# unknownue/puflow

Hardware: AMD Instinct MI355X
Metric: patches/sec x4 2048->8192 (PU1K discrete, eval) (higher is better)
Workload: dtype f32 (split-fp16 MFMA products, fp32 accumulate); 1 GPU; BASELINE configs[1]: PU1K discrete x4 inference, 32 x 2048-pt patches per GPU (fp32-parity mode); patches_per_gpu=32, total_batch=32, npoint=2048

## Files before the change

puflow_amd/csrc/edgeconv.hip:

```cpp
#include <hip/hip_runtime.h>
#include "pf_api_internal.h"
#include "pf_mfma.h"

#if defined(__HIP_DEVICE_COMPILE__)
#define PF_PACKED_FP32_FN __attribute__((target("packed-fp32-ops")))
#else
#define PF_PACKED_FP32_FN
#endif

namespace {

struct EcArgs {
    const float* pq;
    const float* xyz;
    const float* tab;
    const int* idx;
    const f4* wg;
    float* out;
    int T;
    int N;
    int chunk;
    int ntiles;
    const u4* pqf_w;
    const float* pqf_bias;
    const float* pqf_scales;
    float* pqf_out;
};

template <int ODIM>
__device__ __forceinline__ void pqf_stage(u4* hb, int ch, int pt, float v) {
    _Float16* h = reinterpret_cast<_Float16*>(hb);
    const int cp = ch >> 5, j = ((ch >> 4) & 1) * 4 + (ch & 3), slot = 16 * ((ch & 15) >> 2) + pt;
    const _Float16 hi = (_Float16)v;
    const _Float16 lo = (_Float16)(v - (float)hi);
    h[((cp * 2 + 0) * 64 + slot) * 8 + j] = hi;
    h[((cp * 2 + 1) * 64 + slot) * 8 + j] = lo;
}

constexpr int PQF_NT = 4;

template <int ODIM, int ROWS, int NW>
__device__ __forceinline__ void pqf_gemm(const EcArgs& a, const u4* hb, int nst, const int (&tpt)[PQF_NT], int wave_u, int lane) {
    constexpr int CP = ODIM / 32, RB = ROWS / 16 / NW;
    static_assert(ODIM % 32 == 0 && ROWS % (16 * NW) == 0, "rows split evenly over the waves");
    constexpr int OBW = NW <= 8 ? RB : 1;
    const int col = lane & 15, q = lane >> 4;
    const PfW2BufD<CP> ws(a.pqf_w, lane);
    const float inv = a.pqf_scales[6];
#pragma unroll
    for (int ob0 = 0; ob0 < RB; ob0 += OBW) {
        h8 wh[OBW][CP], wl[OBW][CP];
#pragma unroll
        for (int o = 0; o < OBW; ++o)
#pragma unroll
            for (int cp = 0; cp < CP; ++cp) {
                wh[o][cp] = ws.load((wave_u * RB + ob0 + o) * CP + cp, 0);
                wl[o][cp] = ws.load((wave_u * RB + ob0 + o) * CP + cp, 1);
            }
#pragma unroll
        for (int t = 0; t < PQF_NT; ++t) {
            if (t >= nst) break;
            const u4* hbt = hb + t * (CP * 2 * 64);
            f4 acc[OBW];
#pragma unroll
            for (int o = 0; o < OBW; ++o) acc[o] = pf_splat(0.f);
#pragma unroll
            for (int cp = 0; cp < CP; ++cp) {
                const h8 fh = __builtin_bit_cast(h8, hbt[(cp * 2 + 0) * 64 + lane]), fl = __builtin_bit_cast(h8, hbt[(cp * 2 + 1) * 64 + lane]);
#pragma unroll
                for (int o = 0; o < OBW; ++o) {
                    f4 x = acc[o];
                    if constexpr (PF_MMN_TERMS == 3) {
                        x = pf_mfma_f16(wh[o][cp], fl, x);
                        x = pf_mfma_f16(wl[o][cp], fh, x);
                    }
                    x = pf_mfma_f16(wh[o][cp], fh, x);
                    acc[o] = x;
                }
            }
            const int pt = tpt[t] + col;
            if (pt < a.T) {
#pragma unroll
                for (int o = 0; o < OBW; ++o) {
                    const f4 bias = *reinterpret_cast<const f4*>(a.pqf_bias + (wave_u * RB + ob0 + o) * 16 + 4 * q);
                    f4 v;
#pragma unroll
                    for (int r = 0; r < 4; ++r) v[r] = fmaf(acc[o][r], inv, bias[r]);
                    *reinterpret_cast<f4*>(a.pqf_out + (size_t)pt * ROWS + (wave_u * RB + ob0 + o) * 16 + 4 * q) = v;
                }
            }
        }
    }
}

struct PqfState {
    int nst = 0;
    int tpt[PQF_NT] = {0, 0, 0, 0};
    __device__ __forceinline__ void push(int pt0) {
#pragma unroll
        for (int k = 0; k < PQF_NT; ++k) tpt[k] = k == nst ? pt0 : tpt[k];
        ++nst;
    }
};

template <int GB, int NCONV, int ODIM, bool C3, int P, int NW>
__global__ __launch_bounds__(NW * 64) void edgeconv_kernel(EcArgs a) {
    constexpr int G = GB * 16;
    constexpr int S = G * NCONV + ODIM;
    constexpr int NF = GB * NCONV;
    constexpr int OBO = ODIM / 16;
    constexpr int OCH = 2;
    static_assert(OBO <= 16 && OBO % OCH == 0, "pooled store uses one lane column per output block");
    const int lane = threadIdx.x & 63, wave = threadIdx.x >> 6;
    const int col = lane & 15, q = lane >> 4;

    constexpr int NWF = GB * GB * (NCONV * (NCONV - 1) / 2) + OBO * NF;
    __shared__ f4 wlds[NWF * 64];
    pf_stage_lds(wlds, a.wg, NWF * 64);
    __syncthreads();
    const PfWLds ws{wlds, lane};

    for (int v = blockIdx.x; v < 8 * a.chunk; v += gridDim.x) {
        const int tile = pf_xcd_tile(v, a.chunk);
        if (tile >= a.ntiles) continue;
        const int pt0 = (tile * NW + wave) * P;

        int gi[P], gj[P];
        float xi[P][3], xj[P][3];
#pragma unroll
        for (int p = 0; p < P; ++p) {
            int g = pt0 + p;
            g = g < a.T ? g : a.T - 1;
            gi[p] = g;
            const int b = g / a.N;
            gj[p] = b * a.N + a.idx[(size_t)g * 16 + col];
            if constexpr (C3) {
#pragma unroll
                for (int c = 0; c < 3; ++c) {
                    xi[p][c] = a.xyz[(size_t)gi[p] * 3 + c];
                    xj[p][c] = a.xyz[(size_t)gj[p] * 3 + c];
                }
            }
        }

        auto init = [&](int p, int off) -> f4 {
            if constexpr (C3) {
                f4 r;
#pragma unroll
                for (int k = 0; k < 4; ++k) {
                    const f4* t = reinterpret_cast<const f4*>(a.tab + (size_t)(off + k) * 8);
                    const f4 t0 = t[0], t1 = t[1];
                    float s = t1.z;
                    s = fmaf(t0.x, xi[p][0], s); s = fmaf(t0.y, xi[p][1], s); s = fmaf(t0.z, xi[p][2], s);
                    s = fmaf(t0.w, xj[p][0], s); s = fmaf(t1.x, xj[p][1], s); s = fmaf(t1.y, xj[p][2], s);
                    r[k] = s;
                }
                return r;
            } else {
                const f4 pv = *reinterpret_cast<const f4*>(a.pq + (size_t)gi[p] * (2 * S) + off);
                const f4 qv = *reinterpret_cast<const f4*>(a.pq + (size_t)gj[p] * (2 * S) + S + off);
                return pv + qv;
            }
        };

        constexpr int NI = GB > OCH ? GB : OCH;
        f4 ini[2][P][NI];
        auto load_init = [&](auto nbc, int row0, f4 (&dst)[P][NI]) {
            constexpr int NB = decltype(nbc)::value;
#pragma unroll
            for (int ob = 0; ob < NB; ++ob)
#pragma unroll
                for (int p = 0; p < P; ++p) dst[p][ob] = init(p, row0 + ob * 16 + 4 * q);
        };
        using IGB = std::integral_constant<int, GB>;
        using IOC = std::integral_constant<int, OCH>;
        load_init(IGB{}, 0, ini[0]);
        if constexpr (NCONV > 1) load_init(IGB{}, G, ini[1]); else load_init(IOC{}, G * NCONV, ini[1]);

        f4 feat[P][NF];
#pragma unroll
        for (int ob = 0; ob < GB; ++ob)
#pragma unroll
            for (int p = 0; p < P; ++p) feat[p][ob] = pf_lrelu(ini[0][p][ob], 0.05f);

        pf_static_for<1, NCONV>([&](auto tc) {
            constexpr int t = decltype(tc)::value;
            if constexpr (t + 1 < NCONV) load_init(IGB{}, G * (t + 1), ini[(t + 1) & 1]);
            else load_init(IOC{}, G * NCONV, ini[(t + 1) & 1]);
            f4 acc[P][GB];
#pragma unroll
            for (int ob = 0; ob < GB; ++ob)
#pragma unroll
                for (int p = 0; p < P; ++p) acc[p][ob] = ini[t & 1][p][ob];
            pf_mm<GB, GB * t, GB * t>(ws, GB * GB * (t * (t - 1) / 2), feat, 0, acc, 0);
#pragma unroll
            for (int ob = 0; ob < GB; ++ob)
#pragma unroll
                for (int p = 0; p < P; ++p) feat[p][GB * t + ob] = pf_lrelu(acc[p][ob], 0.05f);
        });

        constexpr int FO = GB * GB * (NCONV * (NCONV - 1) / 2);
        f4 sel[P];
#pragma unroll
        for (int p = 0; p < P; ++p) sel[p] = pf_splat(0.f);
        pf_static_for<0, OBO / OCH>([&](auto cc) {
            constexpr int c = decltype(cc)::value;
            constexpr int ob0 = c * OCH;
            constexpr int st = NCONV + c;
            if constexpr (c + 1 < OBO / OCH) load_init(IOC{}, G * NCONV + (ob0 + OCH) * 16, ini[(st + 1) & 1]);
            f4 acc[P][OCH];
#pragma unroll
            for (int o = 0; o < OCH; ++o)
#pragma unroll
                for (int p = 0; p < P; ++p) acc[p][o] = ini[st & 1][p][o];
            pf_mm<OCH, NF, NF>(ws, FO + ob0 * NF, feat, 0, acc, 0);
#pragma unroll
            for (int o = 0; o < OCH; ++o)
#pragma unroll
                for (int p = 0; p < P; ++p) {
                    f4 m;
#pragma unroll
                    for (int r = 0; r < 4; ++r) m[r] = pf_rowmax16(acc[p][o][r]);
                    if (col == ob0 + o) sel[p] = m;
                }
        });
#pragma unroll
        for (int p = 0; p < P; ++p)
            if (col < OBO && pt0 + p < a.T)
                *reinterpret_cast<f4*>(a.out + (size_t)gi[p] * ODIM + col * 16 + 4 * q) = sel[p];
    }
}

struct EcWConst {
    static constexpr int DEPTH = 2;
    int lane;
    __device__ __forceinline__ h8 load(int frag, int split) const {
        const _Float16 x = (_Float16)(float)((lane + frag + split) & 7);
        return (h8){x, x, x, x, x, x, x, x};
    }
};

constexpr float EC4_OUT_INV = 1.f / 256.f;

template <int P, int NW, int DBG = 0, bool PQF = false>
__global__ __launch_bounds__(NW * 64) PF_PACKED_FP32_FN void edgeconv4_kernel(EcArgs a) {
    static_assert(!PQF || NW * P == 16, "the fused P|Q GEMM takes a workgroup tile of 16 points as one MFMA column tile");
    constexpr int NCONV = 4, G = 32, S = 256, OBO = 8, OCH = 2, ODIM = 128;
    constexpr int NWF = 2 * (NCONV * (NCONV - 1) / 2) + OBO * NCONV;
    constexpr int ROWB = 2 * S * 4;
    const int lane = threadIdx.x & 63, wave = threadIdx.x >> 6;
    const int col = lane & 15, q = lane >> 4;
    __shared__ u4 wlds[NWF * 2 * 64];
    __shared__ f4 plds[NW * P][64];
    __shared__ u4 hb[PQF ? PQF_NT * (ODIM / 32) * 2 * 64 : 1];
    PqfState pqf;
    pf_stage_lds(wlds, reinterpret_cast<const u4*>(a.wg), NWF * 2 * 64);
    __syncthreads();
    const PfW2Lds ws_lds{wlds, lane};
    const auto ws = [&] { if constexpr ((DBG & 4) != 0) return EcWConst{lane}; else return ws_lds; }();
    const __amdgpu_buffer_rsrc_t rs = __builtin_amdgcn_make_buffer_rsrc(const_cast<float*>(a.pq), 0, 0x7fffffff, 0x00020000);
    const int blkq = ((q & 1) << 1) | (q >> 1);

    const int vend = 8 * a.chunk;
    auto next_valid = [&](int v) { while (v < vend && pf_xcd_tile(v, a.chunk) >= a.ntiles) v += gridDim.x; return v; };
    struct Pre { int g[P]; int jc[P]; int4 j4[P]; f4 prow[P]; };
    auto fetch = [&](int v, Pre& n) {
        const int pt0 = (pf_xcd_tile(v < vend ? v : blockIdx.x, a.chunk) * NW + wave) * P;
#pragma unroll
        for (int p = 0; p < P; ++p) {
            int g = pt0 + p;
            g = g < a.T ? g : a.T - 1;
            g = __builtin_amdgcn_readfirstlane(g);
            n.g[p] = g;
            n.jc[p] = a.idx[(size_t)g * 16 + col];
            n.j4[p] = *reinterpret_cast<const int4*>(a.idx + (size_t)g * 16 + 4 * q);
            n.prow[p] = __builtin_bit_cast(f4, __builtin_amdgcn_raw_buffer_load_b128(rs, lane * 16, g * ROWB, 0));
        }
    };
    int v = next_valid(blockIdx.x);
    Pre cur;
    if (v < vend) fetch(v, cur);
    while (v < vend) {
        const int pt0 = (pf_xcd_tile(v, a.chunk) * NW + wave) * P;
        const int vn = next_valid(v + gridDim.x);
        int vQ[P];
        int vO[P][4];
        int gout[P];
#pragma unroll
        for (int p = 0; p < P; ++p) {
            const int g = cur.g[p];
            const int bN = (g / a.N) * a.N;
            gout[p] = g;
            plds[wave * P + p][lane] = cur.prow[p];
            vQ[p] = (bN + cur.jc[p]) * ROWB + (S + 4 * q) * 4;
            vO[p][0] = (bN + cur.j4[p].x) * ROWB + (S + G * NCONV + col) * 4;
            vO[p][1] = (bN + cur.j4[p].y) * ROWB + (S + G * NCONV + col) * 4;
            vO[p][2] = (bN + cur.j4[p].z) * ROWB + (S + G * NCONV + col) * 4;
            vO[p][3] = (bN + cur.j4[p].w) * ROWB + (S + G * NCONV + col) * 4;
        }
        fetch(vn, cur);
        auto load_g = [&](int t, f4 (&dst)[P][2]) {
#pragma unroll
            for (int ob = 0; ob < 2; ++ob)
#pragma unroll
                for (int p = 0; p < P; ++p) {
                    const int off = (G * t + 16 * ob) * 4;
                    if constexpr (DBG & 1) { dst[p][ob] = pf_splat((float)(off + vQ[p]) * 1e-9f); continue; }
                    dst[p][ob] = __builtin_bit_cast(f4, __builtin_amdgcn_raw_buffer_load_b128(rs, vQ[p], off, 0));
                }
        };
        auto p_g = [&](int p, int t, int ob) -> f4 { return plds[wave * P + p][(G * t + 16 * ob) / 4 + q]; };
        auto load_o = [&](int ob0, f4 (&dst)[P][2]) {
#pragma unroll
            for (int o = 0; o < OCH; ++o)
#pragma unroll
                for (int p = 0; p < P; ++p)
#pragma unroll
                    for (int r = 0; r < 4; ++r) {
                        if constexpr (DBG & 1) { dst[p][o][r] = (float)(vO[p][r] + ob0 + o) * 1e-9f; continue; }
                        dst[p][o][r] = __builtin_bit_cast(float, __builtin_amdgcn_raw_buffer_load_b32(rs, vO[p][r], (ob0 + o) * 64, 0));
                    }
        };
        f4 ini[2][P][2];
        load_g(0, ini[0]);
        load_g(1, ini[1]);
        PfPairN feat[P][NCONV];
#pragma unroll
        for (int p = 0; p < P; ++p)
            feat[p][0] = pf_pairn(pf_lrelu(ini[0][p][0] + p_g(p, 0, 0), 0.05f), pf_lrelu(ini[0][p][1] + p_g(p, 0, 1), 0.05f));
        pf_static_for<1, NCONV>([&](auto tc) {
            constexpr int t = decltype(tc)::value;
            if constexpr (t + 1 < NCONV) load_g(t + 1, ini[(t + 1) & 1]); else load_o(0, ini[(t + 1) & 1]);
            f4 acc[P][2];
#pragma unroll
            for (int ob = 0; ob < 2; ++ob)
#pragma unroll
                for (int p = 0; p < P; ++p) acc[p][ob] = ini[t & 1][p][ob] + p_g(p, t, ob);
            if constexpr (!(DBG & 2)) pf_mmn<false, 2, t, t>(ws, 2 * (t * (t - 1) / 2), feat, acc);
#pragma unroll
            for (int p = 0; p < P; ++p) {
                if constexpr (DBG & 8) { feat[p][t] = feat[p][0]; feat[p][t].h[0] += (_Float16)acc[p][0].x; continue; }
                feat[p][t] = pf_pairn(pf_lrelu(acc[p][0], 0.05f), pf_lrelu(acc[p][1], 0.05f));
            }
        });
        constexpr int FO = 2 * (NCONV * (NCONV - 1) / 2);
        float m[P][OBO];
        pf_static_for<0, OBO / OCH>([&](auto cc) {
            constexpr int c = decltype(cc)::value;
            constexpr int ob0 = c * OCH;
            constexpr int st = NCONV + c;
            if constexpr (c + 1 < OBO / OCH) load_o(ob0 + OCH, ini[(st + 1) & 1]);
            f4 acc[P][OCH];
#pragma unroll
            for (int o = 0; o < OCH; ++o)
#pragma unroll
                for (int p = 0; p < P; ++p) acc[p][o] = ini[st & 1][p][o];
            if constexpr (!(DBG & 2)) pf_mmn<true, OCH, NCONV, NCONV>(ws, FO + ob0 * NCONV, feat, acc);
#pragma unroll
            for (int o = 0; o < OCH; ++o)
#pragma unroll
                for (int p = 0; p < P; ++p)
                    m[p][ob0 + o] = fmaxf(fmaxf(acc[p][o].x, acc[p][o].y), fmaxf(acc[p][o].z, acc[p][o].w));
        });
#pragma unroll
        for (int p = 0; p < P; ++p) {
            const float o0 = pf_rsmax16(pf_rsmax32(m[p][0], m[p][1]), pf_rsmax32(m[p][2], m[p][3]));
            const float o1 = pf_rsmax16(pf_rsmax32(m[p][4], m[p][5]), pf_rsmax32(m[p][6], m[p][7]));
            const int ch = 16 * blkq + col;
            const float* pr = reinterpret_cast<const float*>(plds[wave * P + p]);
            const float p0 = pr[G * NCONV + ch], p1 = pr[G * NCONV + 64 + ch];
            const float h0 = fmaf(o0, EC4_OUT_INV, p0), h1 = fmaf(o1, EC4_OUT_INV, p1);
            if (pt0 + p < a.T) {
                float* o = a.out + (size_t)gout[p] * ODIM + ch;
                o[0] = h0;
                o[64] = h1;
            }
            if constexpr (PQF) {
                u4* hbt = hb + pqf.nst * ((ODIM / 32) * 2 * 64);
                pqf_stage<ODIM>(hbt, ch, wave * P + p, h0);
                pqf_stage<ODIM>(hbt, ch + 64, wave * P + p, h1);
            }
        }
        if constexpr (PQF) {
            pqf.push(pf_xcd_tile(v, a.chunk) * NW * P);
            if (pqf.nst == PQF_NT || vn >= vend) {
                __syncthreads();
                pqf_gemm<ODIM, 2 * S, NW>(a, hb, pqf.nst, pqf.tpt, __builtin_amdgcn_readfirstlane(wave), lane);
                __syncthreads();
                pqf.nst = 0;
            }
        }
        v = vn;
    }
}

template <int P, int NW, int DBG = 0, bool PQF = false>
int launch4(const EcArgs& a0, hipStream_t s) {
    EcArgs a = a0;
    a.ntiles = (a.T + NW * P - 1) / (NW * P);
    a.chunk = (a.ntiles + 7) / 8;
    int grid = 8 * a.chunk;
    if (grid > 256) grid = 256;
    hipLaunchKernelGGL((edgeconv4_kernel<P, NW, DBG, PQF>), dim3(grid), dim3(NW * 64), 0, s, a);
    return pf_last_launch_status();
}

template <int ODIM, bool C3, int P, int NW, bool PQF = false>
__global__ __launch_bounds__(NW * 64) void edgeconv1n_kernel(EcArgs a) {
    static_assert(!PQF || NW * P == 16, "the fused P|Q GEMM takes a workgroup tile of 16 points as one MFMA column tile");
    constexpr int NCONV = 4, S = 16 * NCONV + ODIM, SB = S / 16, OBO = ODIM / 16;
    constexpr int PQ_ROWS = ODIM == 32 ? 256 : 512;
    constexpr int FO = 4, FT = FO + OBO * 2, NWF = FT + (C3 ? SB / 2 : 0);
    static_assert(!C3 || SB % 2 == 0, "the edge table fills whole 2-KiB slots");
    constexpr int ROWB = 2 * S * 4;
    static_assert(OBO == 2 || OBO == 4, "reduce-scatter below is written for 2 or 4 output blocks");
    const int lane = threadIdx.x & 63, wave = threadIdx.x >> 6;
    const int col = lane & 15, q = lane >> 4;
    __shared__ u4 wlds[NWF * 128];
    __shared__ float plds[C3 ? 1 : NW * P][C3 ? 1 : S];
    __shared__ u4 hb[PQF ? PQF_NT * (ODIM / 32) * 2 * 64 : 1];
    PqfState pqf;
    pf_stage_lds(wlds, reinterpret_cast<const u4*>(a.wg), NWF * 128);
    __syncthreads();
    const PfW2Lds ws{wlds, lane};
    const float inv_tab = C3 ? reinterpret_cast<const float*>(a.wg)[NWF * 512] : 1.f;
    const __amdgpu_buffer_rsrc_t rs = __builtin_amdgcn_make_buffer_rsrc(const_cast<float*>(C3 ? a.xyz : a.pq), 0, 0x7fffffff, 0x00020000);

    for (int v = blockIdx.x; v < 8 * a.chunk; v += gridDim.x) {
        const int tile = pf_xcd_tile(v, a.chunk);
        if (tile >= a.ntiles) continue;
        const int pt0 = (tile * NW + wave) * P;
        int gi[P], vQ[P], vO[P][4];
        h8 e[P];
#pragma unroll
        for (int p = 0; p < P; ++p) {
            int g = pt0 + p;
            g = g < a.T ? g : a.T - 1;
            g = __builtin_amdgcn_readfirstlane(g);
            gi[p] = g;
            const int bN = (g / a.N) * a.N;
            const int jc = bN + a.idx[(size_t)g * 16 + col];
            if constexpr (C3) {
                float xi[3], xj[3];
#pragma unroll
                for (int c = 0; c < 3; ++c) {
                    xi[c] = a.xyz[(size_t)g * 3 + c];
                    xj[c] = a.xyz[(size_t)jc * 3 + c];
                }
                const f4 e0 = {xi[0], xi[1], xi[2], xj[0]}, e1 = {xj[1], xj[2], 0.f, 1.f};
                e[p] = pf_edge_operand(e0, e1, q);
            } else {
                const int4 j4 = *reinterpret_cast<const int4*>(a.idx + (size_t)g * 16 + 4 * q);
                vQ[p] = jc * ROWB + (S + 4 * q) * 4;
                vO[p][0] = (bN + j4.x) * ROWB + (S + 16 * NCONV + col) * 4;
                vO[p][1] = (bN + j4.y) * ROWB + (S + 16 * NCONV + col) * 4;
                vO[p][2] = (bN + j4.z) * ROWB + (S + 16 * NCONV + col) * 4;
                vO[p][3] = (bN + j4.w) * ROWB + (S + 16 * NCONV + col) * 4;
                if (lane * 2 < S) {
                    typedef float f2 __attribute__((ext_vector_type(2)));
                    const f2 pv = *reinterpret_cast<const f2*>(a.pq + (size_t)g * (2 * S) + lane * 2);
                    *reinterpret_cast<f2*>(&plds[wave * P + p][lane * 2]) = pv;
                }
            }
        }
        f4 pre[P][NCONV];
        f4 outi[P][OBO];
        if constexpr (C3) {
#pragma unroll
            for (int p = 0; p < P; ++p) {
#pragma unroll
                for (int b = 0; b < NCONV; ++b) pre[p][b] = pf_splat(0.f);
#pragma unroll
                for (int b = 0; b < OBO; ++b) outi[p][b] = pf_splat(0.f);
            }
            const PfW1Lds wt{wlds + FT * 128, lane};
            pf_mm1<false, NCONV>(wt, 0, e, pre);
            pf_mm1<true, OBO>(wt, NCONV, e, outi);
#pragma unroll
            for (int p = 0; p < P; ++p) {
#pragma unroll
                for (int b = 0; b < NCONV; ++b) pre[p][b] = pre[p][b] * inv_tab;
#pragma unroll
                for (int b = 0; b < OBO; ++b) outi[p][b] = outi[p][b] * inv_tab;
            }
        } else {
#pragma unroll
            for (int b = 0; b < NCONV; ++b)
#pragma unroll
                for (int p = 0; p < P; ++p)
                    pre[p][b] = __builtin_bit_cast(f4, __builtin_amdgcn_raw_buffer_load_b128(rs, vQ[p], b * 64, 0));
#pragma unroll
            for (int b = 0; b < OBO; ++b)
#pragma unroll
                for (int p = 0; p < P; ++p)
#pragma unroll
                    for (int r = 0; r < 4; ++r)
                        outi[p][b][r] = __builtin_bit_cast(float, __builtin_amdgcn_raw_buffer_load_b32(rs, vO[p][r], b * 64, 0));
#pragma unroll
            for (int b = 0; b < NCONV; ++b)
#pragma unroll
                for (int p = 0; p < P; ++p) pre[p][b] += *reinterpret_cast<const f4*>(&plds[wave * P + p][16 * b + 4 * q]);
        }

        PfPairN fp[P][2];
        PfHalfN last[P];
#pragma unroll
        for (int p = 0; p < P; ++p) {
            last[p] = pf_act_halfn(pre[p][0], 0.05f);
            fp[p][0] = pf_join_halfn(last[p], PfHalfN{});
        }
        pf_static_for<1, NCONV>([&](auto tc) {
            constexpr int t = decltype(tc)::value;
            constexpr int CPT = (t + 1) / 2, F0 = (t / 2) * ((t + 1) / 2);
            f4 acc[P][1];
#pragma unroll
            for (int p = 0; p < P; ++p) acc[p][0] = pre[p][t];
            pf_mmn<false, 1, CPT, CPT>(ws, F0, fp, acc);
#pragma unroll
            for (int p = 0; p < P; ++p) {
                const PfHalfN f = pf_act_halfn(acc[p][0], 0.05f);
                if constexpr (t % 2 == 1) fp[p][t / 2] = pf_join_halfn(last[p], f);
                else fp[p][t / 2] = pf_join_halfn(f, PfHalfN{});
                last[p] = f;
            }
        });
        pf_mmn<true, OBO, 2, 2>(ws, FO, fp, outi);
#pragma unroll
        for (int p = 0; p < P; ++p) {
            float m[OBO];
#pragma unroll
            for (int b = 0; b < OBO; ++b) m[b] = fmaxf(fmaxf(outi[p][b].x, outi[p][b].y), fmaxf(outi[p][b].z, outi[p][b].w));
            float o;
            int ch;
            if constexpr (OBO == 4) {
                o = pf_rsmax16(pf_rsmax32(m[0], m[1]), pf_rsmax32(m[2], m[3]));
                ch = 16 * (((q & 1) << 1) | (q >> 1)) + col;
            } else {
                const float n = pf_rsmax32(m[0], m[1]);
                o = pf_rsmax16(n, n);
                ch = 16 * (q >> 1) + col;
            }
            float pv = 0.f;
            if constexpr (!C3) pv = plds[wave * P + p][16 * NCONV + ch];
            const float hv = fmaf(o, EC4_OUT_INV, pv);
            if (pt0 + p < a.T && (OBO == 4 || (q & 1) == 0))
                a.out[(size_t)gi[p] * ODIM + ch] = hv;
            if constexpr (PQF) {
                if (OBO == 4 || (q & 1) == 0) pqf_stage<ODIM>(hb + pqf.nst * ((ODIM / 32) * 2 * 64), ch, wave * P + p, hv);
            }
        }
        if constexpr (PQF) {
            pqf.push(tile * NW * P);
            if (pqf.nst == PQF_NT) {
                __syncthreads();
                pqf_gemm<ODIM, PQ_ROWS, NW>(a, hb, pqf.nst, pqf.tpt, __builtin_amdgcn_readfirstlane(wave), lane);
                __syncthreads();
                pqf.nst = 0;
            }
        }
    }
    if constexpr (PQF) {
        if (pqf.nst > 0) {
            __syncthreads();
            pqf_gemm<ODIM, PQ_ROWS, NW>(a, hb, pqf.nst, pqf.tpt, __builtin_amdgcn_readfirstlane(wave), lane);
        }
    }
}

template <int ODIM, bool C3, int P, int NW, bool PQF = false>
int launch1n(const EcArgs& a0, hipStream_t s) {
    EcArgs a = a0;
    a.ntiles = (a.T + NW * P - 1) / (NW * P);
    a.chunk = (a.ntiles + 7) / 8;
    int grid = 8 * a.chunk;
    const int cap = 256 * (32 / NW);
    if (grid > cap) grid = cap;
    hipLaunchKernelGGL((edgeconv1n_kernel<ODIM, C3, P, NW, PQF>), dim3(grid), dim3(NW * 64), 0, s, a);
    return pf_last_launch_status();
}

template <int ODIM, bool C3>
int launch1n_v(const EcArgs& a, hipStream_t s, int variant) {
    switch (variant) {
        case 1: return launch1n<ODIM, C3, 2, 8>(a, s);
#ifdef PF_TUNING_VARIANTS
        case 0: return launch1n<ODIM, C3, 1, 8>(a, s);
        case 2: return launch1n<ODIM, C3, 1, 16>(a, s);
        case 3: return launch1n<ODIM, C3, 2, 4>(a, s);
#endif
        default: return PF_ERR_UNSUPPORTED;
    }
}

template <int GB, int NCONV, int ODIM, bool C3, int P, int NW>
int launch_v(const EcArgs& a0, hipStream_t s) {
    EcArgs a = a0;
    a.ntiles = (a.T + NW * P - 1) / (NW * P);
    a.chunk = (a.ntiles + 7) / 8;
    constexpr int NF = GB * NCONV;
    constexpr int lds = (GB * GB * (NCONV * (NCONV - 1) / 2) + (ODIM / 16) * NF) * 1024;
    int per_cu = (160 * 1024) / lds;
    const int by_waves = 32 / NW;
    if (per_cu > by_waves) per_cu = by_waves;
    if (per_cu < 1) per_cu = 1;
    int grid = 8 * a.chunk;
    const int cap = 256 * per_cu;
    if (grid > cap) grid = cap;
    hipLaunchKernelGGL((edgeconv_kernel<GB, NCONV, ODIM, C3, P, NW>), dim3(grid), dim3(NW * 64), 0, s, a);
    return pf_last_launch_status();
}

template <int GB, int NCONV, int ODIM, bool C3>
int launch(const EcArgs& a, hipStream_t s, int variant) {
    constexpr int BEST = ODIM == 32 ? 0 : (ODIM == 64 ? 2 : 3);
    if (variant == BEST) {
        if constexpr (BEST == 0) return launch_v<GB, NCONV, ODIM, C3, 2, 8>(a, s);
        else if constexpr (BEST == 2) return launch_v<GB, NCONV, ODIM, C3, 1, 8>(a, s);
        else return launch_v<GB, NCONV, ODIM, C3, 1, 16>(a, s);
    }
#ifdef PF_TUNING_VARIANTS
    switch (variant) {
        case 0: return launch_v<GB, NCONV, ODIM, C3, 2, 8>(a, s);
        case 1: return launch_v<GB, NCONV, ODIM, C3, 2, 4>(a, s);
        case 2: return launch_v<GB, NCONV, ODIM, C3, 1, 8>(a, s);
        case 3: return launch_v<GB, NCONV, ODIM, C3, 1, 16>(a, s);
        default: break;
    }
#endif
    return PF_ERR_UNSUPPORTED;
}

}

extern "C" int pf_edgeconv_tuned(int cfg, int variant, const float* pq_or_xyz, const float* tab, const int* idx,
                                 const float* wfrag, float* out, int B, int N, void* stream) {
    if (!pq_or_xyz || !idx || !wfrag || !out) return PF_ERR_NULL;
    if (B <= 0 || N < 16 || (long long)B * N > (1ll << 30)) return PF_ERR_SHAPE;
    EcArgs a{};
    a.idx = idx; a.wg = reinterpret_cast<const f4*>(wfrag); a.out = out; a.T = B * N; a.N = N;
    hipStream_t s = (hipStream_t)stream;
    switch (cfg) {
        case 0:
            if (!tab) return PF_ERR_NULL;
            a.xyz = pq_or_xyz; a.tab = tab;
            return launch<1, 4, 32, true>(a, s, variant);
        case 1: a.pq = pq_or_xyz; return launch<1, 4, 64, false>(a, s, variant);
        case 2: a.pq = pq_or_xyz; return launch<2, 4, 128, false>(a, s, variant);
        case 7:
            {
                const long long maxT = 0x7fffffffll / 2048;
                if (N > maxT) return PF_ERR_UNSUPPORTED;
                const int Bc = (int)(maxT / N);
                for (int b0 = 0; b0 < B; b0 += Bc) {
                    const int nb = B - b0 < Bc ? B - b0 : Bc;
                    EcArgs c = a;
                    c.pq = pq_or_xyz + (size_t)b0 * N * 512; c.idx = idx + (size_t)b0 * N * 16; c.out = out + (size_t)b0 * N * 128;
                    c.T = nb * N;
                    int rc;
                    switch (variant) {
                        case 0: rc = launch4<1, 16>(c, s); break;
#ifdef PF_TUNING_VARIANTS
                        case 1: rc = launch4<2, 8>(c, s); break;
                        case 2: rc = launch4<1, 8>(c, s); break;
                        case 3: rc = launch4<2, 4>(c, s); break;
                        case 8: rc = launch4<1, 16, 1>(c, s); break;
                        case 9: rc = launch4<1, 16, 2>(c, s); break;
                        case 10: rc = launch4<1, 16, 4>(c, s); break;
                        case 11: rc = launch4<1, 16, 5>(c, s); break;
                        case 12: rc = launch4<1, 16, 3>(c, s); break;
                        case 13: rc = launch4<1, 16, 6>(c, s); break;
                        case 14: rc = launch4<1, 16, 13>(c, s); break;
#endif
                        default: return PF_ERR_UNSUPPORTED;
                    }
                    if (rc != PF_OK) return rc;
                }
                return PF_OK;
            }
        case 8:
            a.xyz = pq_or_xyz;
            if ((long long)B * N * 12 > 0x7fffffffll) return PF_ERR_SHAPE;
            return launch1n_v<32, true>(a, s, variant);
        case 9:
            a.pq = pq_or_xyz;
            if ((long long)B * N * 1024 > 0x7fffffffll) return PF_ERR_SHAPE;
            return launch1n_v<64, false>(a, s, variant);
        default: return PF_ERR_UNSUPPORTED;
    }
}

extern "C" int pf_edgeconv(int cfg, const float* pq_or_xyz, const float* tab, const int* idx, const float* wfrag,
                           float* out, int B, int N, void* stream) {
    static const int best[10] = {0, 2, 3, -1, -1, -1, -1, 0, 1, 1};
    if (cfg < 0 || cfg > 9 || best[cfg] < 0) return PF_ERR_UNSUPPORTED;
    return pf_edgeconv_tuned(cfg, best[cfg], pq_or_xyz, tab, idx, wfrag, out, B, N, stream);
}

extern "C" int pf_edgeconv_pq(int unit, const float* pq_or_xyz, const int* idx, const float* wfrag, float* out, const float* w,
                              const long long* off, float* pq_next, int B, int N, int fuse, void* stream) {
    if (!pq_or_xyz || !idx || !wfrag || !out || !w || !off || !pq_next) return PF_ERR_NULL;
    if (unit < 0 || unit > 4) return PF_ERR_UNSUPPORTED;
    if (B <= 0 || N < 16 || (long long)B * N > (1ll << 30)) return PF_ERR_SHAPE;
    const long long T = (long long)B * N;
    const bool fits32 = unit == 0 ? T * 12 <= 0x7fffffffll : (unit == 1 ? T * 1024 <= 0x7fffffffll : T * 2048 <= 0x7fffffffll);
    const bool fused = fits32 && (fuse == 1 || (fuse < 0 && T <= 16384));
    const int cfg = unit == 0 ? 8 : (unit == 1 ? 9 : 7);
    if (!fused) {
        const int rc = pf_edgeconv(cfg, pq_or_xyz, nullptr, idx, wfrag, out, B, N, stream);
        return rc != PF_OK ? rc : pf_pq_gemm(unit, out, w, off, pq_next, (int)T, stream);
    }
    EcArgs a{};
    a.idx = idx; a.wg = reinterpret_cast<const f4*>(wfrag); a.out = out; a.T = (int)T; a.N = N;
    a.pqf_w = reinterpret_cast<const u4*>(w + off[10]); a.pqf_bias = w + off[11]; a.pqf_scales = w + off[12]; a.pqf_out = pq_next;
    hipStream_t s = (hipStream_t)stream;
    if (unit == 0) { a.xyz = pq_or_xyz; return launch1n<32, true, 2, 8, true>(a, s); }
    a.pq = pq_or_xyz;
    if (unit == 1) return launch1n<64, false, 2, 8, true>(a, s);
    return launch4<1, 16, 0, true>(a, s);
}
```

puflow_amd/interpflow.py:

```python
from __future__ import annotations

import os
from typing import List, Optional, Tuple

import numpy as np
import torch
import torch.nn as nn
from torch import Tensor

from . import _lib
from .packing import COND_CHANNELS, FEAT_CHANNELS, GROWTH, NUM_BLOCKS, fold_state_dict, pack_plan

_EC_CFG = [0, 1, 2, 2, 2, 2]
_CHECK_FINITE = os.environ.get("PF_CHECK_FINITE", "0") == "1"


def _conv_bn(cin: int, cout: int, slope: float) -> nn.Sequential:
    return nn.Sequential(nn.Conv2d(cin, cout, kernel_size=1), nn.BatchNorm2d(cout), nn.LeakyReLU(slope))


class _EdgeConvParams(nn.Module):

    def __init__(self, cin: int, odim: int, growth: int):
        super().__init__()
# ... 104 lines not shown
        self.base = self.blob.data_ptr()
        self.ec_tab0 = pk["ec_tab0"]
        self.ec_w = pk["ec_w"]
        self.ec4_w = pk["ec4_w"]
        self.ec1n_w = pk["ec1n_w"]
        self.post = [_lib.offsets(o) for o in pk["post"]]
        self.post_all = _lib.offsets([v for o in pk["post"] for v in o])
        self.flow = pk["flow"]
        self.interp_off = _lib.offsets(pk["interp"])
        self.ld_const = pk["ld_const"]
        self._logp_ws = {}
        self._side = None
        self.split_interp = 0
        self.fuse_pq = -1

    def _p(self, off: int) -> int:
        return self.base + 4 * off

    def _edgeconv(self, u: int, src: int, idx16: Tensor, h: Tensor, B: int, N: int, s) -> None:
        lib = self.lib
        if self.ec_mode == "f16n":
            w = self.ec1n_w[u] if u < 2 else self.ec4_w[u]
            rc = lib.pf_edgeconv(8 + u if u < 2 else 7, src, None, idx16.data_ptr(), self._p(w), h.data_ptr(), B, N, s)
        else:
            tab = self._p(self.ec_tab0) if u == 0 else None
            rc = lib.pf_edgeconv(_EC_CFG[u], src, tab, idx16.data_ptr(), self._p(self.ec_w[u]), h.data_ptr(), B, N, s)
        _lib.check(rc, f"pf_edgeconv[{self.ec_mode}][{u}]")

    @staticmethod
    def _stream() -> int:
        return torch.cuda.current_stream().cuda_stream

    def knn(self, xyz: Tensor) -> Tensor:
        B, N, _ = xyz.shape
        idx = torch.empty((B, N, 16), dtype=torch.int32, device=xyz.device)
        _lib.check(self.lib.pf_knn(xyz.data_ptr(), xyz.data_ptr(), B, N, N, 16, idx.data_ptr(), None, self._stream()),
                   "pf_knn")
        return idx

    def features(self, xyz: Tensor, idx16: Tensor, want_cs: bool, cs_only: bool = False):
        B, N, _ = xyz.shape
        T, dev, s = B * N, xyz.device, self._stream()
        cp = torch.empty((NUM_BLOCKS, T, 64), dtype=torch.float32, device=dev) if not (cs_only and want_cs) else None
        st = torch.empty((NUM_BLOCKS, T, 8), dtype=torch.float32, device=dev) if not (cs_only and want_cs) else None
        pq = torch.empty((T, 512), dtype=torch.float32, device=dev)
        hs: List[Tensor] = []
        pq2 = torch.empty((T, 512), dtype=torch.float32, device=dev)
        for u in range(NUM_BLOCKS):
            h = torch.empty((T, FEAT_CHANNELS[u + 1]), dtype=torch.float32, device=dev)
            src = xyz.data_ptr() if u == 0 else (pq if u % 2 else pq2).data_ptr()
            nxt = pq2 if u % 2 else pq
            if u + 1 == NUM_BLOCKS:
                self._edgeconv(u, src, idx16, h, B, N, s)
            elif self.ec_mode == "f16n":
                w = self.ec1n_w[u] if u < 2 else self.ec4_w[u]
                _lib.check(self.lib.pf_edgeconv_pq(u, src, idx16.data_ptr(), self._p(w), h.data_ptr(), self.base, self.post[u],
                                                   nxt.data_ptr(), B, N, self.fuse_pq, s), f"pf_edgeconv_pq[{u}]")
            else:
                self._edgeconv(u, src, idx16, h, B, N, s)
                _lib.check(self.lib.pf_pq_gemm(u, h.data_ptr(), self.base, self.post[u], nxt.data_ptr(), T, s), f"pf_pq_gemm[{u}]")
            hs.append(h)
        cs: List[Optional[Tensor]] = [torch.empty((B, N, COND_CHANNELS[u]), dtype=torch.float32, device=dev) if want_cs else None
                                      for u in range(NUM_BLOCKS)]
        self._cond_all(hs, cs if want_cs else None, st, cp, T, s)
        return (cs if want_cs else None), cp, st

    def _cond_all(self, hs, cs, st: Optional[Tensor], cp: Optional[Tensor], T: int, s) -> None:
        import ctypes
        PtrArr = ctypes.c_void_p * NUM_BLOCKS
        h_arr = PtrArr(*[h.data_ptr() for h in hs])
        c_arr = PtrArr(*[c.data_ptr() for c in cs]) if cs is not None else None
        _lib.check(self.lib.pf_cond_all(h_arr, self.base, self.post_all, c_arr, st.data_ptr() if st is not None else None,
                                        cp.data_ptr() if cp is not None else None, T, s), "pf_cond_all")

    def logp_ws(self, B: int, N: int, dev) -> Tensor:
        return torch.zeros((int(self.lib.pf_flow_fwd_logp_ws_floats(B, N)),), dtype=torch.float32, device=dev)

    def flow_f(self, xyz: Tensor, cp: Tensor, st: Tensor, ws: Optional[Tensor] = None):
        B, N, _ = xyz.shape
        T, dev, s = B * N, xyz.device, self._stream()
        z = torch.empty((B, N, 3), dtype=torch.float32, device=dev)
        ld_pt = torch.empty((T,), dtype=torch.float32, device=dev)
        ldj = torch.empty((B,), dtype=torch.float32, device=dev)
        lps = torch.empty((B,), dtype=torch.float32, device=dev)
        logp = torch.empty((), dtype=torch.float32, device=dev)
        if ws is None:
            key = (B, N, s)
            ws = self._logp_ws.get(key)
            if ws is None:
                ws = self._logp_ws[key] = self.logp_ws(B, N, dev)
        _lib.check(self.lib.pf_flow_fwd_logp(xyz.data_ptr(), cp.data_ptr(), st.data_ptr(), self._p(self.flow), z.data_ptr(),
                                             ld_pt.data_ptr(), self.ld_const, B, N, ldj.data_ptr(), lps.data_ptr(), logp.data_ptr(),
                                             ws.data_ptr(), s), "pf_flow_fwd_logp")
        return z, ldj, logp

    def interp(self, xyz: Tensor, z: Tensor, idx16: Tensor, R: int) -> Tensor:
        B, N, _ = xyz.shape
        u = torch.empty((B, N * R, 3), dtype=torch.float32, device=xyz.device)
        _lib.check(self.lib.pf_interp(xyz.data_ptr(), z.data_ptr(), idx16.data_ptr(), self.base, self.interp_off,
                                      u.data_ptr(), B, N, R, self._stream()), "pf_interp")
        return u

    def interp_weights(self, xyz: Tensor, idx16: Tensor) -> Tensor:
        B, N, _ = xyz.shape
        aw = torch.empty((B * N, 8, 4), dtype=torch.float32, device=xyz.device)
        _lib.check(self.lib.pf_interp_weights(xyz.data_ptr(), idx16.data_ptr(), self.base, self.interp_off, aw.data_ptr(), B, N,
                                              self._stream()), "pf_interp_weights")
        return aw

    def flow_g_interp(self, aw: Tensor, z: Tensor, idx16: Tensor, cp: Tensor, st: Tensor, R: int) -> Tensor:
        B, N, _ = z.shape
        x = torch.empty((B, N * R, 3), dtype=torch.float32, device=z.device)
        _lib.check(self.lib.pf_flow_inv_interp(aw.data_ptr(), z.data_ptr(), idx16.data_ptr(), cp.data_ptr(), st.data_ptr(),
                                               self._p(self.flow), x.data_ptr(), B, N, R, self._stream()), "pf_flow_inv_interp")
        return x

    def side_stream(self) -> "torch.cuda.Stream":
        if self._side is None:
            self._side = torch.cuda.Stream(device=self.device)
        return self._side

    def split_interp_for(self, T: int, R: int) -> bool:
        return R <= 4 and self.split_interp == 1

    def flow_g(self, u: Tensor, cp: Tensor, st: Tensor, R: int) -> Tensor:
        B, NR, _ = u.shape
        T = B * NR // R
        x = torch.empty_like(u)
        _lib.check(self.lib.pf_flow_inv(u.data_ptr(), cp.data_ptr(), st.data_ptr(), self._p(self.flow), x.data_ptr(),
                                        T, R, self._stream()), "pf_flow_inv")
        return x


    def profile_stages(self, xyz: Tensor, iters: int = 5, R: int = 4) -> dict:
        B, N, _ = xyz.shape
        T, dev, s = B * N, xyz.device, self._stream()
        acc: dict = {}

        def timed(name, fn):
            a, b = torch.cuda.Event(enable_timing=True), torch.cuda.Event(enable_timing=True)
            a.record()
            r = fn()
            b.record()
            acc.setdefault(name, []).append((a, b))
            return r

        for _ in range(iters + 1):
            idx16 = timed("knn", lambda: self.knn(xyz))
            cp = torch.empty((NUM_BLOCKS, T, 64), dtype=torch.float32, device=dev)
            st = torch.empty((NUM_BLOCKS, T, 8), dtype=torch.float32, device=dev)
            pq = torch.empty((T, 512), dtype=torch.float32, device=dev)
            hs = []
            pq2 = torch.empty((T, 512), dtype=torch.float32, device=dev)
            fused = self.ec_mode == "f16n" and (self.fuse_pq == 1 or (self.fuse_pq < 0 and T <= 16384))
            for u in range(NUM_BLOCKS):
                h = torch.empty((T, FEAT_CHANNELS[u + 1]), dtype=torch.float32, device=dev)
                src = xyz.data_ptr() if u == 0 else (pq if u % 2 else pq2).data_ptr()
                nxt = pq2 if u % 2 else pq
                if fused and u + 1 < NUM_BLOCKS:
                    w = self.ec1n_w[u] if u < 2 else self.ec4_w[u]
                    timed(f"edgeconv{u}+pq", lambda: _lib.check(self.lib.pf_edgeconv_pq(
                        u, src, idx16.data_ptr(), self._p(w), h.data_ptr(), self.base, self.post[u], nxt.data_ptr(), B, N, 1, s)))
                else:
                    timed(f"edgeconv{u}", lambda: self._edgeconv(u, src, idx16, h, B, N, s))
                    if u + 1 < NUM_BLOCKS:
                        timed(f"pq{u}", lambda: _lib.check(self.lib.pf_pq_gemm(u, h.data_ptr(), self.base, self.post[u], nxt.data_ptr(), T, s)))
                hs.append(h)
            timed("cond_all", lambda: self._cond_all(hs, None, st, cp, T, s))
            z, _, _ = timed("flow_f+logp", lambda: self.flow_f(xyz, cp, st))
            u_ = timed("interp", lambda: self.interp(xyz, z, idx16, R))
            timed("flow_g", lambda: self.flow_g(u_, cp, st, R))
        torch.cuda.synchronize()
        return {k: sum(a.elapsed_time(b) for a, b in v[1:]) / (len(v) - 1) for k, v in acc.items()}


class PointInterpFlow(nn.Module):

    def __init__(self, pc_channel: int = 3):
        super().__init__()
        if pc_channel != 3:
            raise ValueError("the HIP path is built for 3-D points (pc_channel=3)")
        self.num_blocks = NUM_BLOCKS
        self.num_neighbors = 16
        self.interp = _InterpParams()
        self.feat_convs = nn.ModuleList(
            [_EdgeConvParams(FEAT_CHANNELS[i], FEAT_CHANNELS[i + 1], GROWTH[i]) for i in range(NUM_BLOCKS)])
        self.merge_convs = nn.ModuleList(
            [_MergeParams(FEAT_CHANNELS[i + 1], COND_CHANNELS[i]) for i in range(NUM_BLOCKS)])
        self.flow_blocks = nn.ModuleList(
            [_FlowBlockParams(pc_channel, 64, COND_CHANNELS[i], i % 2 == 0) for i in range(NUM_BLOCKS)])
        self._engine_cache: Optional[_Engine] = None
        self.sync_batchnorm = False
        self.ec_mode: Optional[str] = None

    def invalidate_plan(self) -> None:
        self._engine_cache = None
        self._sig_tensors = None
        self._plan_gen = getattr(self, "_plan_gen", 0) + 1

    def load_state_dict(self, *a, **kw):
        self.invalidate_plan()
        return super().load_state_dict(*a, **kw)

    def _apply(self, fn, *a, **kw):
        self.invalidate_plan()
        return super()._apply(fn, *a, **kw)

    def _signature(self):
        ts = getattr(self, "_sig_tensors", None)
        if ts is None:
            ts = self._sig_tensors = list(self.parameters()) + list(self.buffers())
        return (tuple([t.data_ptr() for t in ts]), tuple([t._version for t in ts]), getattr(self, "_train_forwards", 0))

    def _engine(self, upratio: int = 4) -> _Engine:
        e = self._engine_cache
        dev = self.flow_blocks[0].actnorm.logs.device
        if e is not None and self._signature() != e.signature:
            self.invalidate_plan()
            e = None
        if e is not None and (e.device != dev or (self.ec_mode is not None and e.ec_mode != self.ec_mode)):
            self.invalidate_plan()
            e = None
        if e is None:
            if dev.type != "cuda":
                raise _lib.PuflowHipError("PointInterpFlow runs on the GPU only: move the module with .to('cuda')")
            e = _Engine(self.state_dict(), dev, self.ec_mode)
            e.signature = self._signature()
            self._engine_cache = e
        return e

    def _check_mode(self):
        if self.training:
            raise RuntimeError("this entry point is eval-only; in train() mode call forward() (differentiable path)")
        for b in self.flow_blocks:
            if not b.actnorm.is_inited:
                raise RuntimeError("ActNorm not initialised: load a checkpoint and call set_to_initialized_state() "
                                   "(reference upsample.py:32-33)")

    @staticmethod
    def _prep(xyz: Tensor) -> Tensor:
        if not xyz.is_cuda:
            raise _lib.PuflowHipError("input must be a GPU tensor (no CPU fallback)")
        return xyz.detach().contiguous().float()

    def set_to_initialized_state(self) -> None:
        for b in self.flow_blocks:
            b.actnorm.is_inited = True

    @torch.no_grad()
    def feat_extract(self, xyz: Tensor, knn_idx: Tensor) -> CondList:
        self._check_mode()
        xyz = self._prep(xyz)
        e = self._engine(4)
        cs, cp, st = e.features(xyz, knn_idx.to(torch.int32).contiguous(), want_cs=True)
        out = CondList(cs)
        out.cp, out.st = cp, st
        return out

    @torch.no_grad()
    def f(self, xyz: Tensor, cs: CondList) -> Tuple[Tensor, Tensor]:
        self._check_mode()
        z, ldj, _ = self._engine(4).flow_f(self._prep(xyz), cs.cp, cs.st)
        return z, ldj

    @torch.no_grad()
    def log_prob(self, xyz: Tensor, cs: CondList) -> Tuple[Tensor, Tensor]:
        self._check_mode()
        z, _, logp = self._engine(4).flow_f(self._prep(xyz), cs.cp, cs.st)
        return z, logp

    @torch.no_grad()
    def g(self, z: Tensor, cs: CondList, upratio: int) -> Tensor:
        self._check_mode()
        u = torch.flatten(self._prep(z).transpose(2, 3), 1, 2).contiguous()
        return self._engine(upratio).flow_g(u, cs.cp, cs.st, upratio)

    def forward(self, xyz: Tensor, upratio: int = 4) -> Tuple[Tensor, Tensor]:
        if self.training:
            from .train_ops import forward_train
            if not xyz.is_cuda:
                raise _lib.PuflowHipError("input must be a GPU tensor (no CPU fallback)")
            self._train_forwards = getattr(self, "_train_forwards", 0) + 1
            return forward_train(self, xyz, upratio)
        with torch.no_grad():
            return self._forward_eval(xyz, upratio)

    def _forward_eval(self, xyz: Tensor, upratio: int, ws: Optional[Tensor] = None) -> Tuple[Tensor, Tensor]:
        self._check_mode()
        xyz = self._prep(xyz)
        e = self._engine(upratio)
        idx16 = e.knn(xyz)
        if e.split_interp_for(xyz.shape[0] * xyz.shape[1], upratio):
            main, side = torch.cuda.current_stream(), e.side_stream()
            side.wait_stream(main)
            with torch.cuda.stream(side):
                aw = e.interp_weights(xyz, idx16)
            _, cp, st = e.features(xyz, idx16, want_cs=False)
            z, _, logp = e.flow_f(xyz, cp, st, ws)
            main.wait_stream(side)
            aw.record_stream(main)
            x = e.flow_g_interp(aw, z, idx16, cp, st, upratio)
        else:
            _, cp, st = e.features(xyz, idx16, want_cs=False)
            z, _, logp = e.flow_f(xyz, cp, st, ws)
            u = e.interp(xyz, z, idx16, upratio)
            x = e.flow_g(u, cp, st, upratio)
        if _CHECK_FINITE and not bool(torch.isfinite(x).all() & torch.isfinite(logp)):
            raise _lib.PuflowHipError("non-finite output: an activation left the fp16 range of the split-fp16 kernels "
                                      "(or the input holds NaN/inf); check the input normalisation (patch.py:168-178)")
        return x, logp

    @torch.no_grad()
    def forward_stages(self, xyz: Tensor, upratio: int = 4) -> dict:
        self._check_mode()
        xyz = self._prep(xyz)
# ... 51 lines not shown
```

Before: 28510 patches/s.

## Fuse P|Q GEMM as a per-block tail pass for large batches

Adds a second fused form in which each edgeconv workgroup, after finishing its own point tiles, runs the next block's P|Q GEMM over those same tiles. It reuses the now-unused weight LDS image as staging for split-fp16 activation tiles and holds the GEMM weights in registers. For large point counts (unit 1 excepted) the default dispatch now picks this form instead of a separate edgeconv launch followed by a standalone pq_gemm launch. The aim is to save a kernel launch and to re-read h while it is likely still cache-resident. The cost is more registers per thread and a serial tail phase at the end of each block. The unit-0/1 kernel also gets a min-waves launch bound for this form.

```diff
diff --git a/puflow_amd/csrc/edgeconv.hip b/puflow_amd/csrc/edgeconv.hip
--- a/puflow_amd/csrc/edgeconv.hip
+++ b/puflow_amd/csrc/edgeconv.hip
@@ -103,6 +103,78 @@
     }
 };
 
+template <int ODIM, int ROWS, int NW, int NT>
+__device__ __forceinline__ void pq_tail(const EcArgs& a, u4* bl, int wave_u, int lane) {
+    constexpr int CP = ODIM / 32, RB = ROWS / 16 / NW, NU = NT * CP;
+    static_assert(ODIM % 32 == 0 && ROWS % (16 * NW) == 0, "rows split evenly over the waves");
+    const int col = lane & 15, q = lane >> 4;
+    const int vend = 8 * a.chunk, vstep = gridDim.x;
+    h8 wh[RB][CP], wl[RB][CP];
+#pragma unroll
+    for (int ob = 0; ob < RB; ++ob)
+#pragma unroll
+        for (int cp = 0; cp < CP; ++cp) {
+            const u4* f = a.pqf_w + (size_t)(((wave_u * RB + ob) * CP + cp) * 2) * 64 + lane;
+            wh[ob][cp] = __builtin_bit_cast(h8, f[0]);
+            wl[ob][cp] = __builtin_bit_cast(h8, f[64]);
+        }
+    const float* biasp = a.pqf_bias + wave_u * RB * 16 + 4 * q;
+    const float inv = a.pqf_scales[6];
+    for (int v0 = blockIdx.x; v0 < vend; v0 += NT * vstep) {
+#pragma unroll
+        for (int u0 = 0; u0 < NU; u0 += NW) {
+            const int u = u0 + wave_u, t = u / CP, cp = u % CP;
+            const int vt = v0 + t * vstep;
+            if (u >= NU || vt >= vend) continue;
+            const int tile = pf_xcd_tile(vt, a.chunk);
+            if (tile >= a.ntiles) continue;
+            int pt = tile * 16 + col;
+            pt = pt < a.T ? pt : tile * 16;
+            const float* hr = a.out + (size_t)pt * ODIM + cp * 32 + 4 * q;
+            const PfPairN p = pf_pairn(*reinterpret_cast<const f4*>(hr), *reinterpret_cast<const f4*>(hr + 16));
+            bl[(u * 2 + 0) * 64 + lane] = __builtin_bit_cast(u4, p.h);
+            bl[(u * 2 + 1) * 64 + lane] = __builtin_bit_cast(u4, p.l);
+        }
+        __syncthreads();
+        for (int t = 0; t < NT; ++t) {
+            const int vt = v0 + t * vstep;
+            if (vt >= vend) break;
+            const int tile = pf_xcd_tile(vt, a.chunk);
+            if (tile >= a.ntiles) continue;
+            const u4* blt = bl + t * (CP * 2 * 64);
+            f4 acc[RB];
+#pragma unroll
+            for (int ob = 0; ob < RB; ++ob) acc[ob] = pf_splat(0.f);
+#pragma unroll
+            for (int cp = 0; cp < CP; ++cp) {
+                const h8 fh = __builtin_bit_cast(h8, blt[(cp * 2 + 0) * 64 + lane]), fl = __builtin_bit_cast(h8, blt[(cp * 2 + 1) * 64 + lane]);
+#pragma unroll
+                for (int ob = 0; ob < RB; ++ob) {
+                    f4 x = acc[ob];
+                    if constexpr (PF_MMN_TERMS == 3) {
+                        x = pf_mfma_f16(wh[ob][cp], fl, x);
+                        x = pf_mfma_f16(wl[ob][cp], fh, x);
+                    }
+                    x = pf_mfma_f16(wh[ob][cp], fh, x);
+                    acc[ob] = x;
+                }
+            }
+            const int pt = tile * 16 + col;
+            if (pt < a.T) {
+#pragma unroll
+                for (int ob = 0; ob < RB; ++ob) {
+                    const f4 bias = *reinterpret_cast<const f4*>(biasp + ob * 16);
+                    f4 o;
+#pragma unroll
+                    for (int r = 0; r < 4; ++r) o[r] = fmaf(acc[ob][r], inv, bias[r]);
+                    *reinterpret_cast<f4*>(a.pqf_out + (size_t)pt * ROWS + (wave_u * RB + ob) * 16 + 4 * q) = o;
+                }
+            }
+        }
+        __syncthreads();
+    }
+}
+
 template <int GB, int NCONV, int ODIM, bool C3, int P, int NW>
 __global__ __launch_bounds__(NW * 64) void edgeconv_kernel(EcArgs a) {
     constexpr int G = GB * 16;
@@ -242,9 +314,9 @@
 
 constexpr float EC4_OUT_INV = 1.f / 256.f;
 
-template <int P, int NW, int DBG = 0, bool PQF = false>
+template <int P, int NW, int DBG = 0, int PQF = 0>
 __global__ __launch_bounds__(NW * 64) PF_PACKED_FP32_FN void edgeconv4_kernel(EcArgs a) {
-    static_assert(!PQF || NW * P == 16, "the fused P|Q GEMM takes a workgroup tile of 16 points as one MFMA column tile");
+    static_assert(PQF == 0 || NW * P == 16, "the fused P|Q GEMM takes a workgroup tile of 16 points as one MFMA column tile");
     constexpr int NCONV = 4, G = 32, S = 256, OBO = 8, OCH = 2, ODIM = 128;
     constexpr int NWF = 2 * (NCONV * (NCONV - 1) / 2) + OBO * NCONV;
     constexpr int ROWB = 2 * S * 4;
@@ -252,7 +324,7 @@
     const int col = lane & 15, q = lane >> 4;
     __shared__ u4 wlds[NWF * 2 * 64];
     __shared__ f4 plds[NW * P][64];
-    __shared__ u4 hb[PQF ? PQF_NT * (ODIM / 32) * 2 * 64 : 1];
+    __shared__ u4 hb[PQF == 1 ? PQF_NT * (ODIM / 32) * 2 * 64 : 1];
     PqfState pqf;
     pf_stage_lds(wlds, reinterpret_cast<const u4*>(a.wg), NWF * 2 * 64);
     __syncthreads();
@@ -375,13 +447,13 @@
                 o[0] = h0;
                 o[64] = h1;
             }
-            if constexpr (PQF) {
+            if constexpr (PQF == 1) {
                 u4* hbt = hb + pqf.nst * ((ODIM / 32) * 2 * 64);
                 pqf_stage<ODIM>(hbt, ch, wave * P + p, h0);
                 pqf_stage<ODIM>(hbt, ch + 64, wave * P + p, h1);
             }
         }
-        if constexpr (PQF) {
+        if constexpr (PQF == 1) {
             pqf.push(pf_xcd_tile(v, a.chunk) * NW * P);
             if (pqf.nst == PQF_NT || vn >= vend) {
                 __syncthreads();
@@ -392,9 +464,15 @@
         }
         v = vn;
     }
-}
-
-template <int P, int NW, int DBG = 0, bool PQF = false>
+    if constexpr (PQF == 2) {
+        constexpr int NT = 8;
+        static_assert(NT * (ODIM / 32) * 2 * 64 <= NWF * 2 * 64, "the staged tiles fit the dead weight image");
+        __syncthreads();
+        pq_tail<ODIM, 2 * S, NW, NT>(a, wlds, __builtin_amdgcn_readfirstlane(wave), lane);
+    }
+}
+
+template <int P, int NW, int DBG = 0, int PQF = 0>
 int launch4(const EcArgs& a0, hipStream_t s) {
     EcArgs a = a0;
     a.ntiles = (a.T + NW * P - 1) / (NW * P);
@@ -405,9 +483,9 @@
     return pf_last_launch_status();
 }
 
-template <int ODIM, bool C3, int P, int NW, bool PQF = false>
-__global__ __launch_bounds__(NW * 64) void edgeconv1n_kernel(EcArgs a) {
-    static_assert(!PQF || NW * P == 16, "the fused P|Q GEMM takes a workgroup tile of 16 points as one MFMA column tile");
+template <int ODIM, bool C3, int P, int NW, int PQF = 0>
+__global__ __launch_bounds__(NW * 64, PQF == 2 ? 4 : 1) void edgeconv1n_kernel(EcArgs a) {
+    static_assert(PQF == 0 || NW * P == 16, "the fused P|Q GEMM takes a workgroup tile of 16 points as one MFMA column tile");
     constexpr int NCONV = 4, S = 16 * NCONV + ODIM, SB = S / 16, OBO = ODIM / 16;
     constexpr int PQ_ROWS = ODIM == 32 ? 256 : 512;
     constexpr int FO = 4, FT = FO + OBO * 2, NWF = FT + (C3 ? SB / 2 : 0);
@@ -418,7 +496,7 @@
     const int col = lane & 15, q = lane >> 4;
     __shared__ u4 wlds[NWF * 128];
     __shared__ float plds[C3 ? 1 : NW * P][C3 ? 1 : S];
-    __shared__ u4 hb[PQF ? PQF_NT * (ODIM / 32) * 2 * 64 : 1];
+    __shared__ u4 hb[PQF == 1 ? PQF_NT * (ODIM / 32) * 2 * 64 : 1];
     PqfState pqf;
     pf_stage_lds(wlds, reinterpret_cast<const u4*>(a.wg), NWF * 128);
     __syncthreads();
@@ -545,11 +623,11 @@
             const float hv = fmaf(o, EC4_OUT_INV, pv);
             if (pt0 + p < a.T && (OBO == 4 || (q & 1) == 0))
                 a.out[(size_t)gi[p] * ODIM + ch] = hv;
-            if constexpr (PQF) {
+            if constexpr (PQF == 1) {
                 if (OBO == 4 || (q & 1) == 0) pqf_stage<ODIM>(hb + pqf.nst * ((ODIM / 32) * 2 * 64), ch, wave * P + p, hv);
             }
         }
-        if constexpr (PQF) {
+        if constexpr (PQF == 1) {
             pqf.push(tile * NW * P);
             if (pqf.nst == PQF_NT) {
                 __syncthreads();
@@ -559,15 +637,21 @@
             }
         }
     }
-    if constexpr (PQF) {
+    if constexpr (PQF == 1) {
         if (pqf.nst > 0) {
             __syncthreads();
             pqf_gemm<ODIM, PQ_ROWS, NW>(a, hb, pqf.nst, pqf.tpt, __builtin_amdgcn_readfirstlane(wave), lane);
         }
     }
-}
-
-template <int ODIM, bool C3, int P, int NW, bool PQF = false>
+    if constexpr (PQF == 2) {
+        constexpr int NT = ODIM == 32 ? 8 : 4;
+        static_assert(NT * (ODIM / 32) * 2 * 64 <= NWF * 128, "the staged tiles fit the dead weight image");
+        __syncthreads();
+        pq_tail<ODIM, PQ_ROWS, NW, NT>(a, wlds, __builtin_amdgcn_readfirstlane(wave), lane);
+    }
+}
+
+template <int ODIM, bool C3, int P, int NW, int PQF = 0>
 int launch1n(const EcArgs& a0, hipStream_t s) {
     EcArgs a = a0;
     a.ntiles = (a.T + NW * P - 1) / (NW * P);
@@ -696,16 +780,18 @@
     return pf_edgeconv_tuned(cfg, best[cfg], pq_or_xyz, tab, idx, wfrag, out, B, N, stream);
 }
 
+constexpr long long PQ_FUSE_MAX_T = 16384;
 extern "C" int pf_edgeconv_pq(int unit, const float* pq_or_xyz, const int* idx, const float* wfrag, float* out, const float* w,
                               const long long* off, float* pq_next, int B, int N, int fuse, void* stream) {
     if (!pq_or_xyz || !idx || !wfrag || !out || !w || !off || !pq_next) return PF_ERR_NULL;
     if (unit < 0 || unit > 4) return PF_ERR_UNSUPPORTED;
     if (B <= 0 || N < 16 || (long long)B * N > (1ll << 30)) return PF_ERR_SHAPE;
+    if (fuse > 2) return PF_ERR_UNSUPPORTED;
     const long long T = (long long)B * N;
     const bool fits32 = unit == 0 ? T * 12 <= 0x7fffffffll : (unit == 1 ? T * 1024 <= 0x7fffffffll : T * 2048 <= 0x7fffffffll);
-    const bool fused = fits32 && (fuse == 1 || (fuse < 0 && T <= 16384));
+    const int form = !fits32 ? 0 : (fuse >= 0 ? fuse : (T <= PQ_FUSE_MAX_T ? 1 : (unit == 1 ? 0 : 2)));
     const int cfg = unit == 0 ? 8 : (unit == 1 ? 9 : 7);
-    if (!fused) {
+    if (form == 0) {
         const int rc = pf_edgeconv(cfg, pq_or_xyz, nullptr, idx, wfrag, out, B, N, stream);
         return rc != PF_OK ? rc : pf_pq_gemm(unit, out, w, off, pq_next, (int)T, stream);
     }
@@ -713,8 +799,8 @@
     a.idx = idx; a.wg = reinterpret_cast<const f4*>(wfrag); a.out = out; a.T = (int)T; a.N = N;
     a.pqf_w = reinterpret_cast<const u4*>(w + off[10]); a.pqf_bias = w + off[11]; a.pqf_scales = w + off[12]; a.pqf_out = pq_next;
     hipStream_t s = (hipStream_t)stream;
-    if (unit == 0) { a.xyz = pq_or_xyz; return launch1n<32, true, 2, 8, true>(a, s); }
+    if (unit == 0) { a.xyz = pq_or_xyz; return form == 1 ? launch1n<32, true, 2, 8, 1>(a, s) : launch1n<32, true, 2, 8, 2>(a, s); }
     a.pq = pq_or_xyz;
-    if (unit == 1) return launch1n<64, false, 2, 8, true>(a, s);
-    return launch4<1, 16, 0, true>(a, s);
-}
+    if (unit == 1) return form == 1 ? launch1n<64, false, 2, 8, 1>(a, s) : launch1n<64, false, 2, 8, 2>(a, s);
+    return form == 1 ? launch4<1, 16, 0, 1>(a, s) : launch4<1, 16, 0, 2>(a, s);
+}
diff --git a/puflow_amd/interpflow.py b/puflow_amd/interpflow.py
--- a/puflow_amd/interpflow.py
+++ b/puflow_amd/interpflow.py
@@ -280,7 +280,7 @@
             pq = torch.empty((T, 512), dtype=torch.float32, device=dev)
             hs = []
             pq2 = torch.empty((T, 512), dtype=torch.float32, device=dev)
-            fused = self.ec_mode == "f16n" and (self.fuse_pq == 1 or (self.fuse_pq < 0 and T <= 16384))
+            fused = self.ec_mode == "f16n" and self.fuse_pq != 0
             for u in range(NUM_BLOCKS):
                 h = torch.empty((T, FEAT_CHANNELS[u + 1]), dtype=torch.float32, device=dev)
                 src = xyz.data_ptr() if u == 0 else (pq if u % 2 else pq2).data_ptr()
@@ -288,7 +288,7 @@
                 if fused and u + 1 < NUM_BLOCKS:
                     w = self.ec1n_w[u] if u < 2 else self.ec4_w[u]
                     timed(f"edgeconv{u}+pq", lambda: _lib.check(self.lib.pf_edgeconv_pq(
-                        u, src, idx16.data_ptr(), self._p(w), h.data_ptr(), self.base, self.post[u], nxt.data_ptr(), B, N, 1, s)))
+                        u, src, idx16.data_ptr(), self._p(w), h.data_ptr(), self.base, self.post[u], nxt.data_ptr(), B, N, self.fuse_pq, s)))
                 else:
                     timed(f"edgeconv{u}", lambda: self._edgeconv(u, src, idx16, h, B, N, s))
                     if u + 1 < NUM_BLOCKS:
```

After: 28810 patches/s (median of 6 runs). +1.1%, better.
